# cedricrommel/manipose

Measured on AMD Instinct MI355X. Metric: train poses/sec (whole node), H36M T=243 J=17 K=5, higher is better.
Workload: dtype bf16x3; 1 GPU; H36M lifting T=243 J=17 K=5 ManiPose full (C=512, depth 8), train step fwd+WTA loss+bwd+allreduce+Adam; windows_per_gpu=158, global_batch=158, seq_len=243, parallelism=dp1, precision=bf16x3, gradient_exchange=none

## Files before the change

### manipose_amd/csrc/attention_mfma.hip

```cpp
#include <stdlib.h>
#include "common.h"
#include "kernels.h"

namespace mp {

typedef short bf16x8_t __attribute__((ext_vector_type(8)));
typedef short bf16x4_t __attribute__((ext_vector_type(4)));
typedef float f32x4 __attribute__((ext_vector_type(4)));

constexpr int TP = 256;
constexpr int NTILE = TP / 16;

__device__ __forceinline__ float sfma(float a, float b, float c) { return __builtin_fmaf(a, b, c); }
__device__ __forceinline__ float sadd(float a, float b) {
#pragma clang fp contract(off)
  return a + b;
}
__device__ __forceinline__ float smul(float a, float b) {
#pragma clang fp contract(off)
  return a * b;
}
__device__ __forceinline__ float ssub(float a, float b) {
#pragma clang fp contract(off)
  return a - b;
// ... 1061 lines not shown
  const int pitch = 6 * C + 16, cpr = (6 * C) >> 4, nchunk = N * cpr;
  char* sh = sm;
  char* sl = sm + N * pitch;
  uint4 pre[2][PER];
  auto fetch = [&](int f) {
    const char* bh = reinterpret_cast<const char*>(qkv_hi + (long)f * N * 3 * C);
    const char* bl = reinterpret_cast<const char*>(qkv_lo + (long)f * N * 3 * C);
#pragma unroll
    for (int i = 0; i < PER; ++i) {
      const int idx = tid + i * nthreads;
      uint4 a = make_uint4(0u, 0u, 0u, 0u), c = a;
      if (idx < nchunk) { a = *reinterpret_cast<const uint4*>(bh + (long)idx * 16); c = *reinterpret_cast<const uint4*>(bl + (long)idx * 16); }
      pre[0][i] = a; pre[1][i] = c;
    }
  };
  auto commit = [&]() {
#pragma unroll
    for (int i = 0; i < PER; ++i) {
      const int idx = tid + i * nthreads, r = idx / cpr, k = idx - r * cpr;
      if (idx < nchunk) {
        *reinterpret_cast<uint4*>(sh + r * pitch + k * 16) = pre[0][i];
        *reinterpret_cast<uint4*>(sl + r * pitch + k * 16) = pre[1][i];
      }
    }
  };
  const int oq = h * D * 2, ok = 2 * C + oq, ov = 4 * C + oq;
  int f = blockIdx.x;
  if (f >= nframes) return;
  fetch(f);
  while (true) {
    __syncthreads();
    commit();
    __syncthreads();
    const int next = f + gridDim.x;
    if (next < nframes) fetch(next);
    bf16x8_t kfh[2][KS], kfl[2][KS];
#pragma unroll
    for (int t = 0; t < 2; ++t)
#pragma unroll
      for (int ks = 0; ks < KS; ++ks) {
        kfh[t][ks] = frag_tok<D>(sh, pitch, ok, 16 * t, ks, lane, N);
        kfl[t][ks] = frag_tok<D>(sl, pitch, ok, 16 * t, ks, lane, N);
      }
    bf16x8_t vTh[DB], vTl[DB];
#pragma unroll
    for (int db = 0; db < DB; ++db) {
      vTh[db] = frag_tokT<D>(sh, pitch, ov, db, lane, N);
      vTl[db] = frag_tokT<D>(sl, pitch, ov, db, lane, N);
    }
#pragma unroll
    for (int qt = 0; qt < 2; ++qt) {
      if (qt * 16 >= N) break;
      bf16x8_t qfh[KS], qfl[KS];
#pragma unroll
      for (int ks = 0; ks < KS; ++ks) {
        qfh[ks] = frag_tok<D>(sh, pitch, oq, 16 * qt, ks, lane, N);
        qfl[ks] = frag_tok<D>(sl, pitch, oq, 16 * qt, ks, lane, N);
      }
      f32x4 s0 = {0.f, 0.f, 0.f, 0.f}, s1 = {0.f, 0.f, 0.f, 0.f};
#pragma unroll
      for (int ks = 0; ks < KS; ++ks) {
        MP_MFMA3(s0, kfh[0][ks], kfl[0][ks], qfh[ks], qfl[ks]);
        MP_MFMA3(s1, kfh[1][ks], kfl[1][ks], qfh[ks], qfl[ks]);
      }
      col_softmax(s0, s1, g, N, scale);
      bf16x8_t bph, bpl;
      pack_acc_x2(s0, s1, bph, bpl);
      const int tq = qt * 16 + l15;
#pragma unroll
      for (int db = 0; db < DB; ++db) {
        f32x4 o = {0.f, 0.f, 0.f, 0.f};
        MP_MFMA3(o, vTh[db], vTl[db], bph, bpl);
        if (tq < N) {
          const long oo = ((long)f * N + tq) * C + h * D + 16 * db + 4 * g;
          store4_o<F8O>(out_hi + oo, out_lo + oo, o, 1.0f);
        }
      }
    }
    if (next >= nframes) break;
    f = next;
  }
}

__global__ void join_planes_kernel(const bf16p* __restrict__ hi, long lo_off, float* __restrict__ out, long n4) {
  const long i = (long)blockIdx.x * blockDim.x + threadIdx.x;
  if (i < n4) st4(out + 4 * i, ld4(hi + 4 * i, lo_off));
}
__global__ void split_planes_kernel(const float* __restrict__ in, bf16p* __restrict__ hi, long lo_off, long n4) {
  const long i = (long)blockIdx.x * blockDim.x + threadIdx.x;
  if (i < n4) st4(hi + 4 * i, ld4(in + 4 * i), lo_off);
}
int join_planes(const bf16* hi, const bf16* lo, float* out, long n, hipStream_t st) {
  MP_CHECK(n % 4 == 0, MP_ERR_ARG, "join_planes: n %% 4");
  hipLaunchKernelGGL(join_planes_kernel, dim3(cdiv(n / 4, 256)), dim3(256), 0, st, reinterpret_cast<const bf16p*>(hi), (long)(lo - hi), out, n / 4);
  MP_LAUNCH_CHECK();
  return MP_OK;
}
int split_planes(const float* in, bf16* hi, bf16* lo, long n, hipStream_t st) {
  MP_CHECK(n % 4 == 0, MP_ERR_ARG, "split_planes: n %% 4");
  hipLaunchKernelGGL(split_planes_kernel, dim3(cdiv(n / 4, 256)), dim3(256), 0, st, in, reinterpret_cast<bf16p*>(hi), (long)(lo - hi), n / 4);
  MP_LAUNCH_CHECK();
  return MP_OK;
}

static int num_cus() {
  static int n = 0;
  if (n == 0) {
    int dev = 0, c = 0;
    if (hipGetDevice(&dev) != hipSuccess || hipDeviceGetAttribute(&c, hipDeviceAttributeMultiprocessorCount, dev) != hipSuccess || c <= 0) c = 256;
    n = c;
  }
  return n;
}
bool attn_x3_needs_scratch(int temporal, int T, int J, int C, int H) {
  const int D = C / H;
  if (temporal) return !(attn_tmfma_supported(T, D) && C % 8 == 0);
  return !(attn_smfma_supported(J, D, H) && C % 8 == 0 && 2L * J * (6 * C + 16) <= 160 * 1024 && (long)J * (6 * C / 16) <= 7L * H * 64);
}

static int fwd_x3_by_fp32(const AttnArgs& a, int temporal, hipStream_t st) {
  const long M = (long)a.B * a.T * a.J;
  int rc = join_planes((const bf16*)a.qkv, (const bf16*)a.qkv_lo, a.scratch, 3 * M * a.C, st);
  if (rc) return rc;
  AttnArgs f = {};
  f.qkv = a.scratch; f.out = a.scratch + 3 * M * a.C; f.lse = a.lse; f.B = a.B; f.T = a.T; f.J = a.J; f.C = a.C; f.H = a.H; f.form = ATTN_F32;
  f.scale = a.scale;
  rc = attn_fwd(f, temporal, st);
  if (rc) return rc;
  return split_planes(a.scratch + 3 * M * a.C, (bf16*)a.out, (bf16*)a.out_lo, M * a.C, st);
}

int attn_spatial_fwd_x3(const AttnArgs& a, hipStream_t st) {
  const int B = a.B, T = a.T, J = a.J, C = a.C, H = a.H, out_f16f8 = a.out_f16f8;
  const bf16 *qkv_hi = (const bf16*)a.qkv, *qkv_lo = (const bf16*)a.qkv_lo;
  bf16 *out_hi = (bf16*)a.out, *out_lo = (bf16*)a.out_lo;
  MP_CHECK(C % H == 0 && C % 4 == 0, MP_ERR_ARG, "attn_spatial_fwd_x3: C=%d H=%d", C, H);
  const int D = C / H;
  MP_CHECK(!out_f16f8 || (D == 64 && !attn_x3_needs_scratch(0, T, J, C, H)), MP_ERR_ARG, "attn_spatial_fwd_x3: f16f8 output needs head dim 64 and the MFMA kernel (J=%d C=%d H=%d)", J, C, H);
  if (attn_x3_needs_scratch(0, T, J, C, H)) {
    MP_CHECK(a.scratch != nullptr, MP_ERR_ARG, "attn_spatial_fwd_x3: J=%d D=%d H=%d needs the fp32 scratch", J, D, H);
    return fwd_x3_by_fp32(a, 0, st);
  }
  const float scale = attn_qk_scale(a.scale, D);
  const size_t lds = 2 * (size_t)J * (6 * C + 16);
  MP_CHECK(lds <= 160 * 1024, MP_ERR_ARG, "attn_spatial_fwd_x3: frame block of %zu bytes exceeds the LDS", lds);
  MP_CHECK((long)J * (6 * C / 16) <= 7L * H * 64, MP_ERR_ARG, "attn_spatial_fwd_x3: frame block too large for the register prefetch (J=%d C=%d H=%d)", J, C, H);
  const int nframes = B * T;
  const int per_cu = (int)max((size_t)1, min((size_t)4, (size_t)(160 * 1024) / lds));
  const int grid = min(nframes, num_cus() * per_cu);
  if (D == 64) {
    static bool attr_set = false;
    if (!attr_set) {
      MP_HIP(hipFuncSetAttribute((const void*)attn_smfma_fwd_x3_kernel<64>, hipFuncAttributeMaxDynamicSharedMemorySize, 160 * 1024));
      attr_set = true;
    }
    if (out_f16f8) {
      static bool attr8_set = false;
      if (!attr8_set) {
        MP_HIP(hipFuncSetAttribute((const void*)attn_smfma_fwd_x3_kernel<64, true>, hipFuncAttributeMaxDynamicSharedMemorySize, 160 * 1024));
        attr8_set = true;
      }
      hipLaunchKernelGGL((attn_smfma_fwd_x3_kernel<64, true>), dim3(grid), dim3(H * 64), lds, st, qkv_hi, qkv_lo, out_hi, out_lo, nframes, J, C, H, scale);
    } else
    hipLaunchKernelGGL(attn_smfma_fwd_x3_kernel<64>, dim3(grid), dim3(H * 64), lds, st, qkv_hi, qkv_lo, out_hi, out_lo, nframes, J, C, H, scale);
  } else {
    static bool attr_set = false;
    if (!attr_set) {
      MP_HIP(hipFuncSetAttribute((const void*)attn_smfma_fwd_x3_kernel<16>, hipFuncAttributeMaxDynamicSharedMemorySize, 160 * 1024));
      attr_set = true;
    }
    hipLaunchKernelGGL(attn_smfma_fwd_x3_kernel<16>, dim3(grid), dim3(H * 64), lds, st, qkv_hi, qkv_lo, out_hi, out_lo, nframes, J, C, H, scale);
  }
  MP_LAUNCH_CHECK();
  return MP_OK;
}

#ifdef ATTN_X3P_NO_FULL
#define ATTN_X3P_FULL_GUARD && false
#else
#define ATTN_X3P_FULL_GUARD
#endif
template <int D, bool F8O = false>
static int launch_tmfma_fwd_x3(const AttnArgs& a, hipStream_t st) {
  const int T = a.T, J = a.J, C = a.C, H = a.H, units = a.B * J * H;
  const bf16 *qkv_hi = (const bf16*)a.qkv, *qkv_lo = (const bf16*)a.qkv_lo;
  bf16 *out_hi = (bf16*)a.out, *out_lo = (bf16*)a.out_lo;
  float* lse = a.lse;
  const float scale = attn_qk_scale(a.scale, D);
  const int ntile = (T + 15) >> 4;
  const int rows = (T + 31) & ~31;
  const int waves = min(8, max((ntile + 1) / 2, cdiv((long)rows * ACfg<D>::CH, 256)));
  const size_t lds = 4 * (size_t)rows * ACfg<D>::ROWB;
  static bool attr_set = false;
  if (!attr_set) {
    MP_HIP(hipFuncSetAttribute((const void*)attn_tmfma_fwd_x3_kernel<D, false, F8O>, hipFuncAttributeMaxDynamicSharedMemorySize, (int)(4 * TP * ACfg<D>::ROWB)));
    MP_HIP(hipFuncSetAttribute((const void*)attn_tmfma_fwd_x3_kernel<D, true, F8O>, hipFuncAttributeMaxDynamicSharedMemorySize, (int)(4 * TP * ACfg<D>::ROWB)));
    attr_set = true;
  }
  const int per_cu = (int)max((size_t)1, min((size_t)4, (size_t)(160 * 1024) / lds));
  const int grid = min(units, num_cus() * per_cu);
#ifdef MP_GEMM_DIAG
  static const int dbg = [] { const char* e = getenv("MANIPOSE_ATTN_DEBUG"); return e ? atoi(e) : 0; }();
#else
  constexpr int dbg = 0;
#endif
  if (ntile == NTILE ATTN_X3P_FULL_GUARD)
    hipLaunchKernelGGL((attn_tmfma_fwd_x3_kernel<D, true, F8O>), dim3(grid), dim3(64 * waves), lds, st, qkv_hi, qkv_lo, out_hi, out_lo, lse, units, T, J, C, H, scale, dbg);
  else
    hipLaunchKernelGGL((attn_tmfma_fwd_x3_kernel<D, false, F8O>), dim3(grid), dim3(64 * waves), lds, st, qkv_hi, qkv_lo, out_hi, out_lo, lse, units, T, J, C, H, scale, dbg);
  MP_LAUNCH_CHECK();
  return MP_OK;
}

int attn_temporal_fwd_x3(const AttnArgs& a, hipStream_t st) {
  const int B = a.B, T = a.T, J = a.J, C = a.C, H = a.H, out_f16f8 = a.out_f16f8;
  MP_CHECK(C % H == 0 && C % 4 == 0, MP_ERR_ARG, "attn_temporal_fwd_x3: C=%d H=%d", C, H);
  const int D = C / H;
  MP_CHECK(!out_f16f8 || (D == 64 && !attn_x3_needs_scratch(1, T, J, C, H)), MP_ERR_ARG, "attn_temporal_fwd_x3: f16f8 output needs head dim 64 and the MFMA kernel (T=%d C=%d H=%d)", T, C, H);
  if (attn_x3_needs_scratch(1, T, J, C, H)) {
    MP_CHECK(a.scratch != nullptr, MP_ERR_ARG, "attn_temporal_fwd_x3: T=%d D=%d needs the fp32 scratch", T, D);
    return fwd_x3_by_fp32(a, 1, st);
  }
  if (D == 64 && T > 128 && (g_attn_two_phase & 1) && (C * 2) % 128 == 0 && (3L * C * 2) % 16 == 0) {
    const bf16 *qkv_hi = (const bf16*)a.qkv, *qkv_lo = (const bf16*)a.qkv_lo;
    bf16 *out_hi = (bf16*)a.out, *out_lo = (bf16*)a.out_lo;
    float* lse = a.lse;
    const float scale = attn_qk_scale(a.scale, D);
    const int units = B * J * H;
    const int rows = (T + 31) & ~31;
    const size_t lds = 4 * (size_t)rows * 128 + 8 * 16 * 144;
// ... 87 lines not shown
```

### manipose_amd/csrc/capi.hip

```cpp
#include <string.h>
#include "common.h"
#include "kernels.h"
#include "../../include/manipose_hip.h"

namespace mp {
const char* last_error();
long wgrad_f32_slab_floats(int Mtok, int Nout, int Kin);
}
using namespace mp;

static LossCfg to_cfg(const mp_loss_config* c) {
  LossCfg l;
  l.beta = c->rmcl_score_reg; l.vel_w = c->vel_loss; l.smooth_w = c->smooth_reg; l.use_joint_weights = c->w_loss; l.squared = c->sq_loss;
  for (int j = 0; j < 17; ++j) l.joint_weights[j] = c->joint_weights[j];
  return l;
}

static int attention_fwd(const char* who, int form, const void* qkv, void* out, float* lse, int temporal, int B, int T, int J, int C, int H,
                         float qk_scale, void* stream) {
  MP_CHECK(qkv && out && (!temporal || lse), MP_ERR_ARG, "%s: null pointer", who);
  MP_CHECK(qk_scale >= 0.f && qk_scale <= 3.0e38f, MP_ERR_ARG, "%s: qk_scale must be finite and >= 0 (0 = head_dim ** -0.5)", who);
  AttnArgs a = {};
  a.qkv = qkv; a.out = out; a.lse = lse; a.B = B; a.T = T; a.J = J; a.C = C; a.H = H; a.form = form; a.scale = qk_scale;
  return attn_fwd(a, temporal, (hipStream_t)stream);
// ... 446 lines not shown
}

int mp_procrustes_errors(const float* pred, const float* gt, const uint8_t* mask, int64_t N, int J, float pred_scale, float gt_scale,
                         float pck_threshold, float auc_max, int auc_steps, float* out, float* scratch, int64_t scratch_floats, void* stream) {
  return procrustes_errors(pred, gt, mask, (long)N, J, pred_scale, gt_scale, pck_threshold, auc_max, auc_steps, 1, out, scratch,
                           (long)scratch_floats, (hipStream_t)stream);
}

int mp_pose_metrics_row_floats(void) { return pose_metrics_row_floats(); }
int mp_bone_length_table(const float* pred, const int64_t* pred_strides, const float* gt, const int64_t* gt_strides, int B, int L, int signed_diff,
                         float* out, void* stream) {
  MP_CHECK(pred && pred_strides && gt && gt_strides && out, MP_ERR_ARG, "mp_bone_length_table: null pointer");
  long ps[4], gs[4];
  for (int i = 0; i < 4; ++i) { ps[i] = (long)pred_strides[i]; gs[i] = (long)gt_strides[i]; }
  return bone_length_table(pred, ps, gt, gs, B, L, signed_diff, out, (hipStream_t)stream);
}
int mp_pose_metrics(const float* pred, const int64_t* pred_strides, const float* gt, const int64_t* gt_strides, const uint8_t* mask, int B,
                    int L, int J, float pred_scale, float gt_scale, float pck_threshold, float auc_max, int auc_steps, int scale_align,
                    float* out, float* len0, float* scratch, int64_t scratch_floats, void* stream) {
  MP_CHECK(pred && pred_strides && out && len0 && scratch, MP_ERR_ARG, "mp_pose_metrics: null pointer");
  long ps[4], gs[4] = {0, 0, 0, 0};
  for (int i = 0; i < 4; ++i) { ps[i] = (long)pred_strides[i]; if (gt_strides) gs[i] = (long)gt_strides[i]; }
  return pose_metrics(pred, ps, gt, gt_strides ? gs : nullptr, mask, B, L, J, pred_scale, gt_scale, pck_threshold, auc_max, auc_steps,
                      scale_align, out, len0, scratch, (long)scratch_floats, (hipStream_t)stream);
}

int64_t mp_bone_extremes_scratch_floats(int64_t frames) { return (int64_t)bone_extremes_scratch_floats((long)frames); }
int mp_bone_extremes(const float* pred, const int64_t* pred_strides, const float* gt, const int64_t* gt_strides, int B, int L, int J,
                     float pred_scale, float gt_scale, int chain, const float* prev_len, int64_t frame_base, float* min_len, float* max_len,
                     float* max_delta, int64_t* max_delta_idx, float* coord_sums, float* last_len, float* scratch, int64_t scratch_floats,
                     void* stream) {
  MP_CHECK(pred && pred_strides, MP_ERR_ARG, "mp_bone_extremes: null pointer");
  long ps[4], gs[4] = {0, 0, 0, 0};
  for (int i = 0; i < 4; ++i) { ps[i] = (long)pred_strides[i]; if (gt_strides) gs[i] = (long)gt_strides[i]; }
  return bone_extremes(pred, ps, gt, gt_strides ? gs : nullptr, B, L, J, pred_scale, gt_scale, chain, prev_len, (long)frame_base, min_len,
                       max_len, max_delta, reinterpret_cast<long*>(max_delta_idx), coord_sums, last_len, scratch, (long)scratch_floats,
                       (hipStream_t)stream);
}

int64_t mp_hypothesis_stats_scratch_floats(int64_t frames) { return (int64_t)hypothesis_stats_scratch_floats((long)frames); }
int mp_hypothesis_stats_row_floats(void) { return hypothesis_stats_row_floats(); }
int mp_hypothesis_stats_row_counts(void) { return hypothesis_stats_row_counts(); }
int mp_hypothesis_stats(const float* poses, const float* scores, const float* target, int B, int K, int T, float pose_scale, float target_scale,
                        float* sums, int64_t* counts, float* jbest_pose, uint8_t* jbest_idx, float* scratch, int64_t scratch_floats,
                        void* stream) {
  return hypothesis_stats(poses, scores, target, B, K, T, pose_scale, target_scale, sums, reinterpret_cast<long*>(counts), jbest_pose, jbest_idx,
                          scratch, (long)scratch_floats, (hipStream_t)stream);
}

int mp_gemm_plan(int M, int N, int K, int form, int epilogue, int cus, int out[4]) {
  MP_CHECK(out, MP_ERR_ARG, "mp_gemm_plan: null out");
  MP_CHECK(M > 0 && N > 0 && K > 0 && cus >= 0, MP_ERR_ARG, "mp_gemm_plan: bad shape M=%d N=%d K=%d cus=%d", M, N, K, cus);
  MP_CHECK(form == GEMM_FORM_BF16 || form == GEMM_FORM_BF16X3 || form == GEMM_FORM_F16F8 || form == GEMM_FORM_F16, MP_ERR_ARG,
           "mp_gemm_plan: form %d (0 bf16, 1 bf16x3, 8 f16f8, 16 fp16)", form);
  MP_CHECK(epilogue >= EPI_BIAS && epilogue <= EPI_SLAB, MP_ERR_ARG, "mp_gemm_plan: epilogue %d", epilogue);
  if (cus == 0) cus = gemm_device_cus();
  MP_CHECK(cus > 0, MP_ERR_HIP, "mp_gemm_plan: no device to ask for its CU count");
  const bool wgrad = epilogue == EPI_SLAB, dgrad = epilogue == EPI_DGELU;
  const GemmPlanIn in = {M, N, K, form, epilogue, wgrad ? 1 : 0, (wgrad || dgrad) ? 1 : 0, 1, wgrad ? (long)M : (long)K, (wgrad || dgrad) ? (long)N : (long)K, 1.0f, cus};
  const GemmPlan pl = gemm_plan(in);
  MP_CHECK(pl.tile != 0, MP_ERR_ARG, "mp_gemm_plan: no kernel of form %d serves M=%d N=%d K=%d with epilogue %d", form, M, N, K, epilogue);
  out[0] = pl.tile; out[1] = pl.persistent; out[2] = pl.workgroups; out[3] = pl.tiles;
  return MP_OK;
}
int mp_gemm_launch_counts(int64_t out[3], int reset) {
  MP_CHECK(out, MP_ERR_ARG, "mp_gemm_launch_counts: null out");
  long long c[3];
  gemm_launch_counts(c, reset);
  for (int i = 0; i < 3; ++i) out[i] = (int64_t)c[i];
  return MP_OK;
}
int mp_set_option(const char* name, int value) {
  MP_CHECK(name, MP_ERR_ARG, "mp_set_option: null name");
  if (!strcmp(name, "gemm_small_tile")) { gemm_bf16_force_small_tile(value != 0); return MP_OK; }
  if (!strcmp(name, "gemm_persist_min_tiles")) { gemm_bf16_persist_min_tiles(value); return MP_OK; }
  if (!strcmp(name, "gemm_persist_mode")) { gemm_bf16_persist_mode(value); return MP_OK; }
  if (!strcmp(name, "gemm_persist_wgs")) { gemm_bf16_persist_wgs(value); return MP_OK; }
  if (!strcmp(name, "gemm_tile")) {
    MP_CHECK(gemm_bf16_tile(value) == MP_OK, MP_ERR_ARG, "mp_set_option: gemm_tile is 0 (planner), 128 or 256, not %d", value);
    return MP_OK;
  }
  if (!strcmp(name, "attn_two_phase")) { attn_two_phase(value); return MP_OK; }
  if (!strcmp(name, "heads_mfma")) { heads_mfma_mode(value); return MP_OK; }
  MP_CHECK(false, MP_ERR_ARG, "mp_set_option: unknown option '%s' (side_streams / f16f8_inputs became mp_model_config::streams / f16f8 in ABI v7)", name);
}

}
```

### manipose_amd/csrc/elementwise.hip

```cpp
#include <stdarg.h>
#include "common.h"
#include "kernels.h"

namespace mp {

static thread_local char g_err[512] = "";
void set_error(const char* fmt, ...) {
  va_list ap;
  va_start(ap, fmt);
  vsnprintf(g_err, sizeof(g_err), fmt, ap);
  va_end(ap);
}
const char* last_error() { return g_err; }

constexpr int LN_MAXV = 4;

template <int V>
__device__ __forceinline__ void row_stats(const float4 (&v)[V], int lane, int C, float eps, float& mean, float& rstd) {
  float s = 0.f;
#pragma unroll
  for (int i = 0; i < V; ++i)
    if (lane * 4 + 256 * i < C) s += (v[i].x + v[i].y) + (v[i].z + v[i].w);
  mean = wave_sum(s) / (float)C;
  float q = 0.f;
// ... 13 lines not shown
  const int nwaves = (gridDim.x * blockDim.x) >> 6;
  const int C = a.C;
  float4 g1[V], b1[V], g2[V], b2[V];
#pragma unroll
  for (int i = 0; i < V; ++i) {
    const int c = lane * 4 + 256 * i;
    const float4 z = make_float4(0.f, 0.f, 0.f, 0.f);
    g1[i] = (a.g1 != nullptr && c < C) ? ld4(a.g1 + c) : z;
    b1[i] = (a.g1 != nullptr && c < C) ? ld4(a.b1 + c) : z;
    g2[i] = (a.g2 != nullptr && c < C) ? ld4(a.g2 + c) : z;
    b2[i] = (a.g2 != nullptr && c < C) ? ld4(a.b2 + c) : z;
  }
  auto load_row = [&](int m, float4 (&v)[V]) {
    const float* xr = a.x + (long)m * C;
#pragma unroll
    for (int i = 0; i < V; ++i) {
      const int c = lane * 4 + 256 * i;
      if (c < C) v[i] = ld4(xr + c);
    }
  };
  auto finish_row = [&](int m, float4 (&v)[V]) {
    if (a.g1 != nullptr) {
      float mean, rstd;
      row_stats<V>(v, lane, C, a.eps1, mean, rstd);
      const float* pr = (a.pos != nullptr) ? a.pos + (long)((m / a.J) % a.T) * C : nullptr;
#pragma unroll
      for (int i = 0; i < V; ++i) {
        const int c = lane * 4 + 256 * i;
        if (c < C) {
          float4 o;
          o.x = (v[i].x - mean) * rstd * g1[i].x + b1[i].x;
          o.y = (v[i].y - mean) * rstd * g1[i].y + b1[i].y;
          o.z = (v[i].z - mean) * rstd * g1[i].z + b1[i].z;
          o.w = (v[i].w - mean) * rstd * g1[i].w + b1[i].w;
          if (pr != nullptr) {
            const float4 p = ld4(pr + c);
            o.x += p.x; o.y += p.y; o.z += p.z; o.w += p.w;
          }
          v[i] = o;
          if (a.x1 != nullptr) st4(a.x1 + (long)m * C + c, o);
        }
      }
      if (lane == 0) {
        a.stats1[2 * (long)m] = mean;
        a.stats1[2 * (long)m + 1] = rstd;
      }
    }
    if (a.g2 != nullptr) {
      float mean, rstd;
      row_stats<V>(v, lane, C, a.eps2, mean, rstd);
      T* yr = reinterpret_cast<T*>(a.y2) + (long)m * C;
      const long lo_off = (a.y2_lo != nullptr && !__is_same(T, f16f8)) ? reinterpret_cast<T*>(a.y2_lo) - reinterpret_cast<T*>(a.y2) : 0;
#pragma unroll
      for (int i = 0; i < V; ++i) {
        const int c = lane * 4 + 256 * i;
        if (c < C) {
          float4 o;
          o.x = (v[i].x - mean) * rstd * g2[i].x + b2[i].x;
          o.y = (v[i].y - mean) * rstd * g2[i].y + b2[i].y;
          o.z = (v[i].z - mean) * rstd * g2[i].z + b2[i].z;
          o.w = (v[i].w - mean) * rstd * g2[i].w + b2[i].w;
          if constexpr (sizeof(T) == 2 && __is_same(T, f16f8)) {
            st4_f16f8(yr + c, reinterpret_cast<char*>(a.y2_lo) + ((long)m * C + c) * 2, o, false);
            if constexpr (B16) st4(reinterpret_cast<bf16*>(a.y2_b16) + (long)m * C + c, o);
          } else st4(yr + c, o, lo_off);
        }
      }
      if (lane == 0) {
        a.stats2[2 * (long)m] = mean;
        a.stats2[2 * (long)m + 1] = rstd;
      }
    }
  };
  for (int m = wave; m < a.M; m += 2 * nwaves) {
    float4 va[V], vb[V];
    const int mb = m + nwaves;
    load_row(m, va);
    if (mb < a.M) load_row(mb, vb);
    finish_row(m, va);
    if (mb < a.M) finish_row(mb, vb);
  }
}

static int row_grid(int M) { return max(1, cdiv(M, 4)); }

int ln_fwd(const LnFwdArgs& a_in, int out_mode, hipStream_t st) {
  LnFwdArgs a = a_in;
  MP_CHECK(a.C % 4 == 0 && a.C <= 256 * LN_MAXV, MP_ERR_ARG, "ln_fwd: C=%d must be a multiple of 4 and <= 1024", a.C);
  MP_CHECK(a.g1 != nullptr || a.g2 != nullptr, MP_ERR_ARG, "ln_fwd: no stage requested");
  MP_CHECK(out_mode < 2 || a.g2 == nullptr || a.y2_lo != nullptr, MP_ERR_ARG, "ln_fwd: planar output without its lo plane");
  MP_CHECK(out_mode != 3 || a.g2 == nullptr || a.C % 64 == 0, MP_ERR_ARG, "ln_fwd: f16f8 output needs C %% 64 == 0");
  if (out_mode < 2) a.y2_lo = nullptr;
#define MP_LN_FWD(TT, V) hipLaunchKernelGGL((ln_fwd_kernel<TT, V>), dim3(row_grid(a.M)), dim3(256), 0, st, a)
#define MP_LN_FWD_V(V) do { if (out_mode == 3 && a.y2_b16 != nullptr) hipLaunchKernelGGL((ln_fwd_kernel<f16f8, V, true>), dim3(row_grid(a.M)), dim3(256), 0, st, a); \
    else if (out_mode == 3) MP_LN_FWD(f16f8, V); else if (out_mode == 2) MP_LN_FWD(bf16p, V); else if (out_mode == 1) MP_LN_FWD(bf16, V); else MP_LN_FWD(float, V); } while (0)
  if (a.C <= 256)      MP_LN_FWD_V(1);
  else if (a.C <= 512) MP_LN_FWD_V(2);
  else                 MP_LN_FWD_V(4);
#undef MP_LN_FWD_V
#undef MP_LN_FWD
  MP_LAUNCH_CHECK();
  return MP_OK;
}

__device__ __forceinline__ unsigned* gs_cnt(const float* gsc) { return reinterpret_cast<unsigned*>(const_cast<float*>(gsc)) + 4; }
#ifndef LNB_GRID_N
#define LNB_GRID_N 1024
#endif
constexpr int LNB_GRID = LNB_GRID_N;

template <typename TDY, int V, int R>
__global__ __launch_bounds__(256) void ln_bwd_kernel(const TDY* __restrict__ dy, const float* __restrict__ x,
                                                      const float* __restrict__ stats, const float* __restrict__ gamma,
                                                      const float* dskip, float* dx, bf16* __restrict__ dx_b16,
                                                      const float* __restrict__ mask, int mask_mode, int T, int J,
                                                      float* __restrict__ partial, int M, int C, float rs, const float* __restrict__ dys_p,
                                                      const float* __restrict__ b16_gs_p) {
  __shared__ float red[4 * 2 * 256 * V];
  const float dys = dys_p != nullptr ? *dys_p : 1.0f, b16_gs = b16_gs_p != nullptr ? *b16_gs_p : 0.f;
  const int lane = threadIdx.x & 63, wv = threadIdx.x >> 6;
  const int wave = (blockIdx.x * blockDim.x + threadIdx.x) >> 6;
  const int nwaves = (gridDim.x * blockDim.x) >> 6;
  float4 dg[V], db[V], gm[V];
#pragma unroll
  for (int i = 0; i < V; ++i) {
    dg[i] = make_float4(0.f, 0.f, 0.f, 0.f);
    db[i] = make_float4(0.f, 0.f, 0.f, 0.f);
    const int c = lane * 4 + 256 * i;
    gm[i] = (c < C) ? ld4(gamma + c) : make_float4(0.f, 0.f, 0.f, 0.f);
  }
  for (int m0 = wave; m0 < M; m0 += R * nwaves) {
    float4 xv[R][V], g[R][V], k[R][V];
    float mean[R], rstd[R], ms[R];
#pragma unroll
    for (int r = 0; r < R; ++r) {
      const int m = m0 + r * nwaves;
      if (m < M) {
        mean[r] = lone(stats[2 * (long)m]);
        rstd[r] = lone(stats[2 * (long)m + 1]);
        ms[r] = (dx_b16 != nullptr) ? droppath_scale(mask, mask_mode, __builtin_amdgcn_readfirstlane(m), T, J) : 1.0f;
#pragma unroll
        for (int i = 0; i < V; ++i) {
          const int c = lane * 4 + 256 * i;
          if (c < C) {
            xv[r][i] = ld4(x + (long)m * C + c);
            g[r][i] = ld4(dy + (long)m * C + c);
            k[r][i] = (dskip != nullptr) ? ld4(dskip + (long)m * C + c) : make_float4(0.f, 0.f, 0.f, 0.f);
          }
        }
      }
    }
#pragma unroll
    for (int r = 0; r < R; ++r) {
      const int m = m0 + r * nwaves;
      if (m >= M) break;
      float4 xh[V], d[V];
      float s1 = 0.f, s2 = 0.f;
#pragma unroll
      for (int i = 0; i < V; ++i) {
        const int c = lane * 4 + 256 * i;
        if (c < C) {
          const float4 gg = make_float4(g[r][i].x * dys, g[r][i].y * dys, g[r][i].z * dys, g[r][i].w * dys);
          xh[i] = make_float4((xv[r][i].x - mean[r]) * rstd[r], (xv[r][i].y - mean[r]) * rstd[r], (xv[r][i].z - mean[r]) * rstd[r],
                              (xv[r][i].w - mean[r]) * rstd[r]);
          dg[i].x += gg.x * xh[i].x; dg[i].y += gg.y * xh[i].y; dg[i].z += gg.z * xh[i].z; dg[i].w += gg.w * xh[i].w;
          db[i].x += gg.x; db[i].y += gg.y; db[i].z += gg.z; db[i].w += gg.w;
          d[i] = make_float4(gg.x * gm[i].x, gg.y * gm[i].y, gg.z * gm[i].z, gg.w * gm[i].w);
          s1 += (d[i].x + d[i].y) + (d[i].z + d[i].w);
          s2 += (d[i].x * xh[i].x + d[i].y * xh[i].y) + (d[i].z * xh[i].z + d[i].w * xh[i].w);
        }
      }
      s1 = wave_sum(s1) / (float)C;
      s2 = wave_sum(s2) / (float)C;
#pragma unroll
      for (int i = 0; i < V; ++i) {
        const int c = lane * 4 + 256 * i;
        if (c < C) {
          float4 o;
          o.x = rstd[r] * (d[i].x - s1 - xh[i].x * s2);
          o.y = rstd[r] * (d[i].y - s1 - xh[i].y * s2);
          o.z = rstd[r] * (d[i].z - s1 - xh[i].z * s2);
// ... 679 lines not shown
```

### manipose_amd/csrc/kernels.h

```cpp
#pragma once
#include "common.h"

namespace mp {

enum { EPI_BIAS = 0, EPI_BIAS_GELU = 1, EPI_BIAS_RESID = 2, EPI_DGELU = 3, EPI_SLAB = 4 };
struct GemmF32Args {
  const float* A;
  const float* B;
  float* C;
  long lda, ldb, ldc;
  int M, N, K;
  const float* bias;
  float* Z;
  const float* R;
  const float* mask;
  float rscale;
  int mask_mode, T, J;
  float* bias_slab;
  int k_per_split;
};
int gemm_f32(int AL, int BL, int EPI, GemmF32Args g, hipStream_t st);
int wgrad_f32(const float* dY, long lddy, const float* X, long ldx, int Mtok, int Nout, int Kin, float* dW, float* db,
              float* slab, long slab_floats, hipStream_t st);

struct GemmB16Args {
  const void* A;
  const void* B;
  void* C;
  long lda, ldb, ldc;
  int M, N, K;
  const float* bias;
  void* Z;
  const float* R;
  const float* rstats;
  const float* rgamma;
  const float* rbeta;
  const float* mask;
  int mask_mode, T, J;
  float* bias_slab;
  int bias_parts;
  int k_per_split;
  int debug;
  int stagger;
  long long* stamps;
  const void* A_lo;
  const void* B_lo;
  void* C_lo;
  float rscale;
  int f16;
  int out_f16f8;
  const float* gout;
  unsigned* gsat;
};
int gemm_bf16(GemmB16Args g, int a_f32, int a_tr, int b_tr, int c_f32, int epi, hipStream_t st);
int gemm_bf16x3(GemmB16Args g, int c_f32, int epi, hipStream_t st);
int gemm_f16f8(GemmB16Args g, int c_f32, int epi, hipStream_t st);
int cast_to_f16f8(const float* src, void* hi16, void* cat8, long n, int weight, hipStream_t st);
int cast_to_bf16x2(const float* src, bf16* hi, bf16* lo, long n, hipStream_t st);
int wgrad_bf16(const void* dY, int dy_f32, long lddy, const bf16* X, long ldx, int Mtok, int Nout, int Kin, float* dW, float* db,
               float* slab, long slab_floats, hipStream_t st, int f16 = 0, const float* oscale = nullptr, int x_f16 = 0);
int cast_to_bf16(const float* src, bf16* dst, long n, hipStream_t st);
enum { GEMM_FORM_BF16 = 0, GEMM_FORM_BF16X3 = 1, GEMM_FORM_F16F8 = 8, GEMM_FORM_F16 = 16 };
struct GemmPlanIn {
  int M, N, K;
  int form;
  int epi;
  int tra, trb;
  int splits;
  long lda, ldb;
  float rscale;
  int cus;
};
struct GemmPlan {
  int tile;
  int persistent;
  int workgroups;
  int tiles;
};
GemmPlan gemm_plan(const GemmPlanIn& p);
int gemm_device_cus();
int gemm_bf16_tile(int tile);
void gemm_launch_counts(long long out[3], int reset);
void gemm_bf16_force_small_tile(bool on);
void gemm_bf16_persist_min_tiles(int n);
void gemm_bf16_persist_mode(int mode);
void gemm_bf16_persist_wgs(int n);
int gemm_bf16_take_last_persist();

struct LnFwdArgs {
  const float* x;
  int M, C;
  const float* g1; const float* b1; float eps1;
  const float* pos; int T, J;
  float* x1; float* stats1;
  const float* g2; const float* b2; float eps2;
  void* y2; float* stats2;
  void* y2_lo;
  void* y2_b16;
};
int ln_fwd(const LnFwdArgs& a, int out_mode , hipStream_t st);
int ln_bwd(const void* dy, int dy_bf16, const float* x, const float* stats, const float* gamma, const float* dskip, float* dx, void* dx_b16,
           const float* mask, int mask_mode, int T, int J, float* dgamma, float* dbeta, int M, int C, float* scratch,
           long scratch_floats, hipStream_t st, hipStream_t st_param = nullptr, hipEvent_t ev = nullptr, float rs = 1.0f,
           const float* dy_scale = nullptr, const float* b16_gs = nullptr);
int ln_bwd2(const void* dy1, int dy_bf16, const float* x1, const float* stats1, const float* gamma1, const float* dskip,
            const float* x0, const float* stats0, const float* gamma0, const float* beta0 ,
            float* dx, void* dx_b16, const float* mask, int mask_mode, int T, int J, float* dgamma1, float* dbeta1, float* dgamma0, float* dbeta0, int M, int C, float* scratch, long scratch_floats,
            hipStream_t st, hipStream_t st_param = nullptr, hipEvent_t ev = nullptr, float rs = 1.0f, const float* dy_scale = nullptr,
            const float* b16_gs = nullptr);
int grad_scale(const float* d_poses, long n_poses, const float* d_scores, long n_scores, float* gsc, hipStream_t st);
int grad_health_pack(const float* gsc, float* out4, hipStream_t st);
int scale_copy(float* dst, const float* src, float s, long n, hipStream_t st);
int axpy_scaled(float* dst, const float* src, float s, long n, hipStream_t st);

int embed_fwd(const float* xin, const float* W, const float* b, const float* spos, float* out, int M, int C, int J,
              hipStream_t st);
long embed_bwd_scratch_floats(int C, int J);
int embed_bwd(const float* g, const float* xin, float* dW, float* db, float* dspos, int M, int C, int J, float* scratch,
              long scratch_floats, hipStream_t st);
int bones_embed_fwd(const float* xin, const float* W, const float* b, const float* spos, float* out, int BT, int IN, int O,
                    hipStream_t st);
int bones_embed_bwd(const float* g, const float* xin, float* dW, float* db, float* dspos, int BT, int IN, int O,
                    float* scratch, long scratch_floats, hipStream_t st);
int tpos_grad(const float* g, float* dtpos, int B, int T, int J, int C, hipStream_t st);
int scale_rows(const float* g, const float* mask, int mask_mode, void* out, int out_bf16, int M, int C, int T, int J, hipStream_t st);
int adam_step(float* p, const float* g, float* m, float* v, long n, int step, float lr, float beta1, float beta2, float eps,
              float weight_decay, float grad_scale, hipStream_t st, const float* lr_mult = nullptr, const float* wd_mult = nullptr);
struct MaskDesc { int offset, count; float keep; };
int droppath_masks(float* masks, const MaskDesc* descs, int ndesc, unsigned long long seed, unsigned long long step,
                   hipStream_t st);

enum { ATTN_F32 = 0, ATTN_BF16 = 1, ATTN_BF16X3 = 2 };
struct AttnArgs {
  const void* qkv;
  const void* qkv_lo;
  void* out;
  void* out_lo;
  const void* dout;
  void* dqkv;
  float* lse;
  float* delta;
  float* scratch;
  int B, T, J, C, H;
  int form;
  float scale;
  const float* grad_f16;
  int out_f16;
  int out_f16f8;
};
inline float attn_qk_scale(float scale, int D) { return scale > 0.f ? scale : 1.0f / sqrtf((float)D); }
int attn_fwd(const AttnArgs& a, int temporal, hipStream_t st);
int attn_bwd(const AttnArgs& a, int temporal, hipStream_t st);
bool attn_tmfma_supported(int T, int D);
bool attn_smfma_supported(int N, int D, int H);
bool attn_x3_needs_scratch(int temporal, int T, int J, int C, int H);
int attn_smfma_fwd(const AttnArgs& a, hipStream_t st);
int attn_smfma_bwd(const AttnArgs& a, hipStream_t st);
int attn_tmfma_fwd(const AttnArgs& a, hipStream_t st);
int attn_tmfma_bwd(const AttnArgs& a, hipStream_t st);
int attn_spatial_fwd_x3(const AttnArgs& a, hipStream_t st);
int attn_temporal_fwd_x3(const AttnArgs& a, hipStream_t st);
void attn_two_phase(int on);
int join_planes(const bf16* hi, const bf16* lo, float* out, long n, hipStream_t st);
int split_planes(const float* in, bf16* hi, bf16* lo, long n, hipStream_t st);

struct HeadParams { const float* gamma[8]; const float* beta[8]; const float* W[8]; const float* b[8]; };
struct HeadGrads { float* gamma[8]; float* beta[8]; float* W[8]; float* b[8]; };
int heads_fwd(const float* x, const HeadParams& p, int K, int O, float* out, float* stats, int M, int C, hipStream_t st);
bool heads_mfma_supported(int K, int O, int C);
inline long heads_fold_floats(int C) { return 48L * C + 48; }
bool heads_use_mfma(int K, int O, int C);
void heads_mfma_mode(int mode);
int heads_fwd_mfma(const float* x, const HeadParams& p, int K, int O, float* out, float* stats, int M, int C, float* fold, hipStream_t st);
int heads_bwd_mfma(const float* x, const float* stats, const float* fold, const float* out, const HeadParams& p, const HeadGrads& gp, int K, int O,
                   const float* dout, float* dx, int M, int C, float* scratch, long scratch_floats, hipStream_t st, hipStream_t st_param);
int heads_bwd(const float* x, const float* stats, const HeadParams& p, const HeadGrads& gp, int K, int O, const float* dout,
              float* dx, int M, int C, float* scratch, long scratch_floats, hipStream_t st, hipStream_t st_param = nullptr);
struct ScoreParams { const float* w[8]; const float* b[8]; };
struct ScoreGrads { float* w[8]; float* b[8]; };
int scores_fwd(const float* headout, const ScoreParams& p, int K, int O, float* scores, int B, int T, int J, hipStream_t st);
long scores_bwd_scratch_floats(int K, int B, int T);
int scores_bwd(const float* headout, const float* scores, const float* dscores, const ScoreParams& p, const ScoreGrads& gp,
               int K, int O, float* dheadout, int B, int T, int J, float* scratch, long scratch_floats, hipStream_t st, hipStream_t st_param = nullptr, hipEvent_t ev = nullptr);
// ... 51 lines not shown
```

Measured before the change: 129,900 poses/s.

## Add per-wave spatial attention kernel and row-per-wave LayerNorm forward

Adds a spatial attention forward kernel in which each wave handles one (frame, head) unit. The wave DMAs that head's Q/K/V slices straight into LDS with an XOR swizzle and reads V with transposed LDS loads, replacing the old frame-per-workgroup persistent kernel. Separately adds a LayerNorm forward kernel that processes one row per wave, loading gamma/beta per row, used whenever a first affine is present. Both are on by default behind a new 'stream_forms' option; the aim is finer-grained parallelism and less LDS pressure, at the cost of redundant K/V fragment loads and more blocks.

```diff
diff --git a/manipose_amd/csrc/attention_mfma.hip b/manipose_amd/csrc/attention_mfma.hip
--- a/manipose_amd/csrc/attention_mfma.hip
+++ b/manipose_amd/csrc/attention_mfma.hip
@@ -1167,6 +1167,124 @@
   }
 }
 
+constexpr int SW_ROWB = 384, SW_WAVES = 4;
+template <int ROWB>
+__device__ __forceinline__ bf16x8_t frag_tok_sw(const char* __restrict__ S, int seg, int tok0, int ks, int lane, int N) {
+  const int g = lane >> 4, tok = min(tok0 + (lane & 15), N - 1);
+  return *reinterpret_cast<const bf16x8_t*>(S + tok * ROWB + seg * 128 + (((4 * ks + g) ^ (tok & 7)) << 4));
+}
+template <int ROWB>
+__device__ __forceinline__ bf16x8_t frag_tokT_sw(const char* __restrict__ S, int seg, int db, int lane, int N) {
+  typedef bf16x4_t __attribute__((address_space(3))) * lds_ptr;
+  const int li = lane & 15, q = li >> 2, p = li & 3, g = lane >> 4;
+  const int r1 = min(4 * g + q, N - 1), r2 = min(16 + 4 * g + q, N - 1);
+  const int ch = 2 * db + (p >> 1), sub = seg * 128 + (p & 1) * 8;
+  const bf16x4_t lo = __builtin_amdgcn_ds_read_tr16_b64_v4i16((lds_ptr)(S + r1 * ROWB + sub + ((ch ^ (r1 & 7)) << 4)));
+  const bf16x4_t hi = __builtin_amdgcn_ds_read_tr16_b64_v4i16((lds_ptr)(S + r2 * ROWB + sub + ((ch ^ (r2 & 7)) << 4)));
+  bf16x8_t f;
+  f[0] = lo[0]; f[1] = lo[1]; f[2] = lo[2]; f[3] = lo[3]; f[4] = hi[0]; f[5] = hi[1]; f[6] = hi[2]; f[7] = hi[3];
+  return f;
+}
+template <int NSEG>
+__device__ __forceinline__ void sw_dma_lines(char* S, const char* __restrict__ base, long tok_bytes, long seg_bytes, int N, int lane) {
+  typedef __attribute__((address_space(3))) void* lptr;
+  typedef const __attribute__((address_space(1))) void* gptr;
+  const int nchunk = N * NSEG * 8;
+  for (int i = 0; i * 64 < nchunk; ++i) {
+    const int idx = lane + 64 * i;
+    if (idx < nchunk) {
+      const int r = idx / (NSEG * 8), k = idx - r * (NSEG * 8), seg = k >> 3, c = (k & 7) ^ (r & 7);
+      __builtin_amdgcn_global_load_lds((gptr)(base + r * tok_bytes + seg * seg_bytes + c * 16), (lptr)(S + i * 1024), 16, 0, 0);
+    }
+  }
+}
+template <bool FUSE0>
+__device__ __forceinline__ void col_softmax_w(f32x4& s0, f32x4& s1, int g, int N, float scale) {
+#pragma clang fp contract(off)
+  const float raw0 = s0[0];
+  float mx = -INFINITY;
+#pragma unroll
+  for (int r = 0; r < 4; ++r) {
+    s0[r] = (4 * g + r < N) ? s0[r] * scale : -INFINITY;
+    s1[r] = (16 + 4 * g + r < N) ? s1[r] * scale : -INFINITY;
+    mx = fmaxf(mx, fmaxf(s0[r], s1[r]));
+  }
+  mx = group_max(mx);
+  float sum = 0.f;
+#pragma unroll
+  for (int r = 0; r < 4; ++r) {
+    s0[r] = __expf((FUSE0 && r == 0) ? __builtin_fmaf(raw0, scale, -mx) : s0[r] - mx);
+    s1[r] = __expf(s1[r] - mx);
+    sum += s0[r] + s1[r];
+  }
+  const float inv = 1.0f / group_sum(sum);
+#pragma unroll
+  for (int r = 0; r < 4; ++r) { s0[r] *= inv; s1[r] *= inv; }
+}
+template <bool F8O>
+__global__ __launch_bounds__(SW_WAVES * 64) void attn_smfma_fwd_x3_wave_kernel(const bf16* __restrict__ qkv_hi, const bf16* __restrict__ qkv_lo,
+                                                                               bf16* __restrict__ out_hi, bf16* __restrict__ out_lo, int nunits, int N,
+                                                                               int C, int H, float scale) {
+  extern __shared__ __attribute__((aligned(16))) char sm[];
+  constexpr int D = 64, KS = ACfg<D>::KS, DB = ACfg<D>::DB;
+  const int lane = threadIdx.x & 63, w = __builtin_amdgcn_readfirstlane((int)(threadIdx.x >> 6));
+  const int g = lane >> 4, l15 = lane & 15;
+  const int u = blockIdx.x * SW_WAVES + w;
+  if (u >= nunits) return;
+  const int f = u / H, h = u - f * H;
+  const int plane = N * SW_ROWB;
+  char* const sh = sm + w * 2 * plane;
+  char* const sl = sh + plane;
+  sw_dma_lines<3>(sh, reinterpret_cast<const char*>(qkv_hi + (long)f * N * 3 * C + h * D), 6L * C, 2L * C, N, lane);
+  sw_dma_lines<3>(sl, reinterpret_cast<const char*>(qkv_lo + (long)f * N * 3 * C + h * D), 6L * C, 2L * C, N, lane);
+  __builtin_amdgcn_s_waitcnt(0x0070);
+  asm volatile("" ::: "memory");
+  bf16x8_t kfh[2][KS], kfl[2][KS];
+#pragma unroll
+  for (int t = 0; t < 2; ++t)
+#pragma unroll
+    for (int ks = 0; ks < KS; ++ks) {
+      kfh[t][ks] = frag_tok_sw<SW_ROWB>(sh, 1, 16 * t, ks, lane, N);
+      kfl[t][ks] = frag_tok_sw<SW_ROWB>(sl, 1, 16 * t, ks, lane, N);
+    }
+  bf16x8_t vTh[DB], vTl[DB];
+#pragma unroll
+  for (int db = 0; db < DB; ++db) {
+    vTh[db] = frag_tokT_sw<SW_ROWB>(sh, 2, db, lane, N);
+    vTl[db] = frag_tokT_sw<SW_ROWB>(sl, 2, db, lane, N);
+  }
+#pragma unroll
+  for (int qt = 0; qt < 2; ++qt) {
+    if (qt * 16 >= N) break;
+    bf16x8_t qfh[KS], qfl[KS];
+#pragma unroll
+    for (int ks = 0; ks < KS; ++ks) {
+      qfh[ks] = frag_tok_sw<SW_ROWB>(sh, 0, 16 * qt, ks, lane, N);
+      qfl[ks] = frag_tok_sw<SW_ROWB>(sl, 0, 16 * qt, ks, lane, N);
+    }
+    f32x4 s0 = {0.f, 0.f, 0.f, 0.f}, s1 = {0.f, 0.f, 0.f, 0.f};
+#pragma unroll
+    for (int ks = 0; ks < KS; ++ks) {
+      MP_MFMA3(s0, kfh[0][ks], kfl[0][ks], qfh[ks], qfl[ks]);
+      MP_MFMA3(s1, kfh[1][ks], kfl[1][ks], qfh[ks], qfl[ks]);
+    }
+    if (qt == 0) col_softmax_w<false>(s0, s1, g, N, scale);
+    else col_softmax_w<true>(s0, s1, g, N, scale);
+    bf16x8_t bph, bpl;
+    pack_acc_x2(s0, s1, bph, bpl);
+    const int tq = qt * 16 + l15;
+#pragma unroll
+    for (int db = 0; db < DB; ++db) {
+      f32x4 o = {0.f, 0.f, 0.f, 0.f};
+      MP_MFMA3(o, vTh[db], vTl[db], bph, bpl);
+      if (tq < N) {
+        const long oo = ((long)f * N + tq) * C + h * D + 16 * db + 4 * g;
+        store4_o<F8O>(out_hi + oo, out_lo + oo, o, 1.0f);
+      }
+    }
+  }
+}
+
 __global__ void join_planes_kernel(const bf16p* __restrict__ hi, long lo_off, float* __restrict__ out, long n4) {
   const long i = (long)blockIdx.x * blockDim.x + threadIdx.x;
   if (i < n4) st4(out + 4 * i, ld4(hi + 4 * i, lo_off));
@@ -1231,6 +1349,21 @@
   MP_CHECK(lds <= 160 * 1024, MP_ERR_ARG, "attn_spatial_fwd_x3: frame block of %zu bytes exceeds the LDS", lds);
   MP_CHECK((long)J * (6 * C / 16) <= 7L * H * 64, MP_ERR_ARG, "attn_spatial_fwd_x3: frame block too large for the register prefetch (J=%d C=%d H=%d)", J, C, H);
   const int nframes = B * T;
+  if (D == 64 && stream_forms_on()) {
+    const size_t wlds = (size_t)SW_WAVES * 2 * J * SW_ROWB;
+    MP_CHECK((long)nframes * H < (1L << 31) - SW_WAVES, MP_ERR_ARG, "attn_spatial_fwd_x3: %d frames x %d heads exceed the unit index", nframes, H);
+    static bool wattr_set = false;
+    if (!wattr_set) {
+      MP_HIP(hipFuncSetAttribute((const void*)attn_smfma_fwd_x3_wave_kernel<false>, hipFuncAttributeMaxDynamicSharedMemorySize, 160 * 1024));
+      MP_HIP(hipFuncSetAttribute((const void*)attn_smfma_fwd_x3_wave_kernel<true>, hipFuncAttributeMaxDynamicSharedMemorySize, 160 * 1024));
+      wattr_set = true;
+    }
+    const int units = nframes * H, wgrid = cdiv(units, SW_WAVES);
+    if (out_f16f8) hipLaunchKernelGGL(attn_smfma_fwd_x3_wave_kernel<true>, dim3(wgrid), dim3(SW_WAVES * 64), wlds, st, qkv_hi, qkv_lo, out_hi, out_lo, units, J, C, H, scale);
+    else hipLaunchKernelGGL(attn_smfma_fwd_x3_wave_kernel<false>, dim3(wgrid), dim3(SW_WAVES * 64), wlds, st, qkv_hi, qkv_lo, out_hi, out_lo, units, J, C, H, scale);
+    MP_LAUNCH_CHECK();
+    return MP_OK;
+  }
   const int per_cu = (int)max((size_t)1, min((size_t)4, (size_t)(160 * 1024) / lds));
   const int grid = min(nframes, num_cus() * per_cu);
   if (D == 64) {
diff --git a/manipose_amd/csrc/capi.hip b/manipose_amd/csrc/capi.hip
--- a/manipose_amd/csrc/capi.hip
+++ b/manipose_amd/csrc/capi.hip
@@ -552,6 +552,7 @@
   }
   if (!strcmp(name, "attn_two_phase")) { attn_two_phase(value); return MP_OK; }
   if (!strcmp(name, "heads_mfma")) { heads_mfma_mode(value); return MP_OK; }
+  if (!strcmp(name, "stream_forms")) { stream_forms(value); return MP_OK; }
   MP_CHECK(false, MP_ERR_ARG, "mp_set_option: unknown option '%s' (side_streams / f16f8_inputs became mp_model_config::streams / f16f8 in ABI v7)", name);
 }
 
diff --git a/manipose_amd/csrc/elementwise.hip b/manipose_amd/csrc/elementwise.hip
--- a/manipose_amd/csrc/elementwise.hip
+++ b/manipose_amd/csrc/elementwise.hip
@@ -119,7 +119,89 @@
   }
 }
 
+template <typename T, int V, bool B16 = false>
+__global__ __launch_bounds__(256) void ln_fwd_row_kernel(LnFwdArgs a) {
+  const int lane = threadIdx.x & 63;
+  const int m = __builtin_amdgcn_readfirstlane((int)((blockIdx.x * blockDim.x + threadIdx.x) >> 6));
+  if (m >= a.M) return;
+  const int C = a.C;
+  float4 v[V], gm[V], bt[V];
+  {
+    const float* xr = a.x + (long)m * C;
+#pragma unroll
+    for (int i = 0; i < V; ++i) {
+      const int c = lane * 4 + 256 * i;
+      if (c < C) v[i] = ld4(xr + c);
+    }
+  }
+  auto load_affine = [&](const float* gp, const float* bp) {
+#pragma unroll
+    for (int i = 0; i < V; ++i) {
+      const int c = lane * 4 + 256 * i;
+      const float4 z = make_float4(0.f, 0.f, 0.f, 0.f);
+      gm[i] = (c < C) ? ld4(gp + c) : z;
+      bt[i] = (c < C) ? ld4(bp + c) : z;
+    }
+  };
+  {
+    load_affine(a.g1, a.b1);
+    float mean, rstd;
+    row_stats<V>(v, lane, C, a.eps1, mean, rstd);
+    const float* pr = (a.pos != nullptr) ? a.pos + (long)((m / a.J) % a.T) * C : nullptr;
+#pragma unroll
+    for (int i = 0; i < V; ++i) {
+      const int c = lane * 4 + 256 * i;
+      if (c < C) {
+        float4 o;
+        o.x = (v[i].x - mean) * rstd * gm[i].x + bt[i].x;
+        o.y = (v[i].y - mean) * rstd * gm[i].y + bt[i].y;
+        o.z = (v[i].z - mean) * rstd * gm[i].z + bt[i].z;
+        o.w = (v[i].w - mean) * rstd * gm[i].w + bt[i].w;
+        if (pr != nullptr) {
+          const float4 p = ld4(pr + c);
+          o.x += p.x; o.y += p.y; o.z += p.z; o.w += p.w;
+        }
+        v[i] = o;
+        if (a.x1 != nullptr) st4(a.x1 + (long)m * C + c, o);
+      }
+    }
+    if (lane == 0) {
+      a.stats1[2 * (long)m] = mean;
+      a.stats1[2 * (long)m + 1] = rstd;
+    }
+    if (a.g2 == nullptr) return;
+  }
+  load_affine(a.g2, a.b2);
+  float mean, rstd;
+  row_stats<V>(v, lane, C, a.eps2, mean, rstd);
+  T* yr = reinterpret_cast<T*>(a.y2) + (long)m * C;
+  const long lo_off = (a.y2_lo != nullptr && !__is_same(T, f16f8)) ? reinterpret_cast<T*>(a.y2_lo) - reinterpret_cast<T*>(a.y2) : 0;
+#pragma unroll
+  for (int i = 0; i < V; ++i) {
+    const int c = lane * 4 + 256 * i;
+    if (c < C) {
+      float4 o;
+      o.x = (v[i].x - mean) * rstd * gm[i].x + bt[i].x;
+      o.y = (v[i].y - mean) * rstd * gm[i].y + bt[i].y;
+      o.z = (v[i].z - mean) * rstd * gm[i].z + bt[i].z;
+      o.w = (v[i].w - mean) * rstd * gm[i].w + bt[i].w;
+      if constexpr (sizeof(T) == 2 && __is_same(T, f16f8)) {
+        st4_f16f8(yr + c, reinterpret_cast<char*>(a.y2_lo) + ((long)m * C + c) * 2, o, false);
+        if constexpr (B16) st4(reinterpret_cast<bf16*>(a.y2_b16) + (long)m * C + c, o);
+      } else st4(yr + c, o, lo_off);
+    }
+  }
+  if (lane == 0) {
+    a.stats2[2 * (long)m] = mean;
+    a.stats2[2 * (long)m + 1] = rstd;
+  }
+}
+
 static int row_grid(int M) { return max(1, cdiv(M, 4)); }
+
+static int g_stream_forms = 1;
+void stream_forms(int on) { g_stream_forms = on != 0; }
+int stream_forms_on() { return g_stream_forms; }
 
 int ln_fwd(const LnFwdArgs& a_in, int out_mode, hipStream_t st) {
   LnFwdArgs a = a_in;
@@ -131,9 +213,20 @@
 #define MP_LN_FWD(TT, V) hipLaunchKernelGGL((ln_fwd_kernel<TT, V>), dim3(row_grid(a.M)), dim3(256), 0, st, a)
 #define MP_LN_FWD_V(V) do { if (out_mode == 3 && a.y2_b16 != nullptr) hipLaunchKernelGGL((ln_fwd_kernel<f16f8, V, true>), dim3(row_grid(a.M)), dim3(256), 0, st, a); \
     else if (out_mode == 3) MP_LN_FWD(f16f8, V); else if (out_mode == 2) MP_LN_FWD(bf16p, V); else if (out_mode == 1) MP_LN_FWD(bf16, V); else MP_LN_FWD(float, V); } while (0)
-  if (a.C <= 256)      MP_LN_FWD_V(1);
-  else if (a.C <= 512) MP_LN_FWD_V(2);
-  else                 MP_LN_FWD_V(4);
+#define MP_LN_ROW(TT, V, B16) hipLaunchKernelGGL((ln_fwd_row_kernel<TT, V, B16>), dim3(row_grid(a.M)), dim3(256), 0, st, a)
+#define MP_LN_ROW_V(V) do { if (out_mode == 3 && a.y2_b16 != nullptr) MP_LN_ROW(f16f8, V, true); else if (out_mode == 3) MP_LN_ROW(f16f8, V, false); \
+    else if (out_mode == 2) MP_LN_ROW(bf16p, V, false); else if (out_mode == 1) MP_LN_ROW(bf16, V, false); else MP_LN_ROW(float, V, false); } while (0)
+  if (g_stream_forms && a.g1 != nullptr) {
+    if (a.C <= 256)      MP_LN_ROW_V(1);
+    else if (a.C <= 512) MP_LN_ROW_V(2);
+    else                 MP_LN_ROW_V(4);
+  } else {
+    if (a.C <= 256)      MP_LN_FWD_V(1);
+    else if (a.C <= 512) MP_LN_FWD_V(2);
+    else                 MP_LN_FWD_V(4);
+  }
+#undef MP_LN_ROW_V
+#undef MP_LN_ROW
 #undef MP_LN_FWD_V
 #undef MP_LN_FWD
   MP_LAUNCH_CHECK();
diff --git a/manipose_amd/csrc/kernels.h b/manipose_amd/csrc/kernels.h
--- a/manipose_amd/csrc/kernels.h
+++ b/manipose_amd/csrc/kernels.h
@@ -99,6 +99,8 @@
   void* y2_b16;
 };
 int ln_fwd(const LnFwdArgs& a, int out_mode , hipStream_t st);
+void stream_forms(int on);
+int stream_forms_on();
 int ln_bwd(const void* dy, int dy_bf16, const float* x, const float* stats, const float* gamma, const float* dskip, float* dx, void* dx_b16,
            const float* mask, int mask_mode, int T, int J, float* dgamma, float* dbeta, int M, int C, float* scratch,
            long scratch_floats, hipStream_t st, hipStream_t st_param = nullptr, hipEvent_t ev = nullptr, float rs = 1.0f,
```

New measurement: 130,800 poses/s, median of 6. No clear change (+0.7%).
